# felipeagc/sycl-ray-tracer

Hardware: AMD Instinct MI355X
Metric: Mrays/s (higher is better)
Workload: dtype f32

## Files before the change

### include/rt_mi355x.h

```cpp
#ifndef RT_MI355X_H
#define RT_MI355X_H

#include <stddef.h>
#include <stdint.h>

#ifdef __cplusplus
extern "C" {
#endif

#define RT_ABI_VERSION 8

typedef enum rt_status {
    RT_OK = 0,
    RT_ERR_INVALID = -1,
    RT_ERR_NO_DEVICE = -2,
    RT_ERR_HIP = -3,
    RT_ERR_OOM = -4,
    RT_ERR_UNSUPPORTED = -5
} rt_status;

#define RT_TEX_SIZE 512u
#define RT_TEX_CHANNELS 4u
#define RT_TEX_MAX_LAYERS 128u

// ... 432 lines not shown
const void* rt_comm_frame_f32(const rt_comm* c);
const void* rt_comm_frame_u8(const rt_comm* c);

int rt_probe_xorshift(int device, uint32_t seed, uint32_t n, float* out, uint32_t* state_out);
int rt_probe_half_roundtrip(int device, uint32_t n, const float* in, float* out,
                            uint16_t* bits_out);
int rt_probe_scatter(rt_scene* scene, uint32_t material, uint32_t n, const float* dir,
                     const float* normal, const float* uv, const uint32_t* seed, uint8_t* ok,
                     float* out_dir, float* out_att, uint32_t* seed_out);

int rt_probe_rounding(int device, uint64_t* mismatches);

int rt_probe_origin_skip(int device, uint32_t n, const uint32_t* entries, const float* org, const float* dir,
                         uint32_t* word_device, uint32_t* word_host);

const char* rt_last_error(void);
int rt_abi_version(void);
int rt_device_count(void);

#ifdef __cplusplus
}
#endif
#endif
```

### sycl-ray-tracer_amd/csrc/rt_bounce.h

```cpp
#pragma once
#include "rt_device.h"

namespace rt {

RT_DEV f3 ray_dir(const RayState& r) { return mk3(h2f(r.dir[0]), h2f(r.dir[1]), h2f(r.dir[2])); }

template <bool FROM_TRAV = false, class Sink = NoSink>
RT_DEV bool shade_bounce(const SceneDev& S, uint32_t& rng, RayState& r, const Hit& h, f3& result, const Trav* T = nullptr, const ShadeTables* tab = nullptr,
                         long long* ck = nullptr, const Sink& sink = Sink{}) {
    f3 org = FROM_TRAV ? T->o : r.org;
    f3 dir = FROM_TRAV ? T->d : ray_dir(r);
    f3 att = mk3(h2f(r.att[0]), h2f(r.att[1]), h2f(r.att[2]));
    f3 rad = mk3(h2f(r.rad[0]), h2f(r.rad[1]), h2f(r.rad[2]));
    const bool done = FROM_TRAV ? shade_hit<true>(S, *tab, rng, h, org, dir, att, rad, result, ck, sink) : shade_hit<false>(S, ShadeTables{}, rng, h, org, dir, att, rad, result, nullptr, sink);
    r.org = org;
    r.dir[0] = f2h(dir.x), r.dir[1] = f2h(dir.y), r.dir[2] = f2h(dir.z);
    r.att[0] = f2h(att.x), r.att[1] = f2h(att.y), r.att[2] = f2h(att.z);
    r.rad[0] = f2h(rad.x), r.rad[1] = f2h(rad.y), r.rad[2] = f2h(rad.z);
    return done;
}

RT_DEV void origin_skip_none(const TravStack& stack) { *lds_at(skip_word_addr(stack)) = (int32_t)kSkipNone; }
RT_DEV SkipRec skip_entry(const SkipRec* at) {
    const u32x4* ep = reinterpret_cast<const u32x4*>(at);
    const u32x4 a = ep[0], b = ep[1];
    SkipRec e;
    e.ref = a.x, e.n[0] = __uint_as_float(a.y), e.n[1] = __uint_as_float(a.z), e.n[2] = __uint_as_float(a.w);
    e.p[0] = __uint_as_float(b.x), e.p[1] = __uint_as_float(b.y), e.p[2] = __uint_as_float(b.z), e.a = b.w;
    return e;
}
RT_DEV void origin_skip(const SceneDev& S, uint32_t tri, const Trav& T, const TravStack& stack) {
    const SkipRec e = skip_entry(S.skip + (tri == kNoTri ? 0u : tri));
    const float o[3] = {T.o.x, T.o.y, T.o.z}, d[3] = {T.d.x, T.d.y, T.d.z};
    const uint32_t w = origin_skip_word(e, o, d);
    *lds_at(skip_word_addr(stack)) = (int32_t)(tri == kNoTri ? kSkipNone : w);
}

RT_DEV bool roulette(uint32_t& rng, RayState& r) {
    const float qx = h2f(r.att[0]), qy = h2f(r.att[1]), qz = h2f(r.att[2]);
    const float p = __builtin_fminf(__builtin_fmaxf(__builtin_fmaxf(qx, __builtin_fmaxf(qy, qz)), 0.05f), 1.0f);
    const float u = rng_next(rng);
    if (!(u < p)) return false;
    r.att[0] = f2h(qx / p), r.att[1] = f2h(qy / p), r.att[2] = f2h(qz / p);
    return true;
}

}
```

### sycl-ray-tracer_amd/csrc/rt_device.h

```cpp
#pragma once
#include <hip/hip_runtime.h>

#include "../../include/rt_mi355x.h"
#include "rt_types.h"

namespace rt {

#define RT_DEV __device__ __forceinline__

struct f3 {
    float x, y, z;
};
RT_DEV f3 mk3(float x, float y, float z) { return f3{x, y, z}; }
RT_DEV f3 operator+(f3 a, f3 b) { return mk3(a.x + b.x, a.y + b.y, a.z + b.z); }
RT_DEV f3 operator-(f3 a, f3 b) { return mk3(a.x - b.x, a.y - b.y, a.z - b.z); }
RT_DEV f3 operator-(f3 a) { return mk3(-a.x, -a.y, -a.z); }
RT_DEV f3 operator*(f3 a, f3 b) { return mk3(a.x * b.x, a.y * b.y, a.z * b.z); }
RT_DEV f3 operator*(float s, f3 a) { return mk3(s * a.x, s * a.y, s * a.z); }
RT_DEV f3 operator*(f3 a, float s) { return mk3(a.x * s, a.y * s, a.z * s); }
RT_DEV float dot3(f3 a, f3 b) { return (a.x * b.x + a.y * b.y) + a.z * b.z; }
RT_DEV f3 cross3(f3 a, f3 b) {
    return mk3(a.y * b.z - a.z * b.y, a.z * b.x - a.x * b.z, a.x * b.y - a.y * b.x);
}
RT_DEV float rcp_rn(float x) {
// ... 132 lines not shown

constexpr int32_t kTravDone = (int32_t)0x80000000;
#if defined(RT_DEVELOPER_KNOBS) && defined(RT_VOTE_INNER) && defined(RT_VOTE_LEAF)
constexpr uint32_t kVoteInner = RT_VOTE_INNER, kVoteLeaf = RT_VOTE_LEAF;
#else
constexpr uint32_t kVoteInner = 3u, kVoteLeaf = 4u;
#endif
struct Trav {
    f3 o, d;
    float ix, iy, iz;
    float ox, oy, oz;
    Hit best;
    int32_t cur;
    uint32_t sp;
};

struct TravStack;
RT_DEV uint32_t stack_base(const TravStack& st);
RT_DEV void trav_begin(Trav& T, f3 o, f3 d, const TravStack& st) {
    T.o = o, T.d = d;
    T.best.t = __builtin_huge_valf();
    T.best.u = T.best.v = 0.0f;
    T.best.tri = kNoTri;
    const float kTiny = 1e-30f;
    const float dx = __builtin_fabsf(d.x) < kTiny ? __builtin_copysignf(kTiny, d.x) : d.x;
    const float dy = __builtin_fabsf(d.y) < kTiny ? __builtin_copysignf(kTiny, d.y) : d.y;
    const float dz = __builtin_fabsf(d.z) < kTiny ? __builtin_copysignf(kTiny, d.z) : d.z;
    T.ix = __builtin_amdgcn_rcpf(dx), T.iy = __builtin_amdgcn_rcpf(dy), T.iz = __builtin_amdgcn_rcpf(dz);
    T.ox = -o.x * T.ix, T.oy = -o.y * T.iy, T.oz = -o.z * T.iz;
    T.cur = 0;
// ... 66 lines not shown

struct TravSigns {
    lmask nx, ny, nz;
};

RT_DEV float ub0(uint32_t w) { return (float)(w & 0xffu); }
RT_DEV float ub1(uint32_t w) { return (float)((w >> 8) & 0xffu); }
RT_DEV float ub2(uint32_t w) { return (float)((w >> 16) & 0xffu); }
RT_DEV float ub3(uint32_t w) { return (float)(w >> 24); }

struct WaveStats {
    uint32_t inner_steps = 0, inner_lanes = 0, leaf_steps = 0, leaf_lanes = 0;
    uint32_t shade_rounds = 0, shade_lanes = 0, live_lane_steps = 0, top_lanes = 0;
};
RT_DEV TravSigns trav_signs(const Trav& T) { return TravSigns{lanes(T.ix < 0.0f), lanes(T.iy < 0.0f), lanes(T.iz < 0.0f)}; }
template <bool SKIP = false, bool MISS_KEYS = false>
RT_DEV void trav_inner(const SceneDev& S, Trav& T, const TravStack& stack, const TopTree& top, const TravSigns& sg) {
    const float inf = __builtin_huge_valf();
    uint32_t skip = kSkipNone;
    if (SKIP) skip = (uint32_t)*lds_at(skip_word_addr(stack));
    float k0, k1, k2, k3;
    u32x4 w0, w1, w2, chw;
    if (T.cur < top.count * 64) {
        const uint32_t o = (uint32_t)T.cur >> 2;
        w0 = *(lds_u32x4*)(size_t)((uint32_t)(size_t)top.w0 + o), w1 = *(lds_u32x4*)(size_t)((uint32_t)(size_t)top.w1 + o);
        w2 = *(lds_u32x4*)(size_t)((uint32_t)(size_t)top.w2 + o), chw = *(lds_u32x4*)(size_t)((uint32_t)(size_t)top.ch + o);
    } else {
        asm volatile("global_load_dwordx4 %0, %4, %5\n\t"
                     "global_load_dwordx4 %1, %4, %5 offset:16\n\t"
                     "global_load_dwordx4 %2, %4, %5 offset:32\n\t"
                     "global_load_dwordx4 %3, %4, %5 offset:48"
                     : "=&v"(w0), "=&v"(w1), "=&v"(w2), "=&v"(chw)
                     : "v"((uint32_t)T.cur), "s"(S.nodes)
                     : "memory");
    }
// ... 111 lines not shown
        tri_test(S.tris + (size_t)first * kTriBytes, T.o, T.d, T.best);
        if (rem) T.cur = ~(int32_t)(((first + 1u) << 2) | (rem - 1u));
        else trav_pop(T, stack);
    }
}

struct TravClasses {
    lmask inner, leaf;
};
RT_DEV lmask trav_done(const Trav& T) { return lanes(T.cur == kTravDone); }
RT_DEV TravClasses trav_classes(const Trav& T) { return TravClasses{lanes(T.cur >= 0), lanes((uint32_t)T.cur > (uint32_t)kTravDone)}; }
RT_DEV TravClasses trav_classes(const Trav& T, lmask done) {
    const lmask inner = lanes(T.cur >= 0);
    return TravClasses{inner, lanes(true) & ~(inner | done)};
}
template <bool STATS = false, bool LEAF_BATCH = false, bool SKIP = false, bool MISS_KEYS = false>
RT_DEV uint32_t trav_step_wave(const SceneDev& S, Trav& T, const TravStack& stack, const TopTree& top, const TravSigns& sg, const TravClasses& c, WaveStats* ws = nullptr) {
    const uint32_t ni = count(c.inner), nl = count(c.leaf);
    if (ni * kVoteInner >= nl * kVoteLeaf && !(LEAF_BATCH && nl >= 64u)) {
        if (STATS && ni) ws->inner_steps++, ws->inner_lanes += ni, ws->top_lanes += count(c.inner & lanes(T.cur < (SKIP ? top.count : kTopNodes) * 64));
        if (in_mask(c.inner)) trav_inner<SKIP, MISS_KEYS>(S, T, stack, top, sg);
    } else {
        if (STATS) ws->leaf_steps++, ws->leaf_lanes += nl;
        if (in_mask(c.leaf)) trav_leaf<LEAF_BATCH>(S, T, stack);
    }
    return ni + nl;
}
template <bool STATS = false, bool LEAF_BATCH = false, bool SKIP = false, bool MISS_KEYS = false>
RT_DEV uint32_t trav_step_wave(const SceneDev& S, Trav& T, const TravStack& stack, const TopTree& top, const TravSigns& sg, WaveStats* ws = nullptr) {
    return trav_step_wave<STATS, LEAF_BATCH, SKIP, MISS_KEYS>(S, T, stack, top, sg, trav_classes(T), ws);
}

RT_DEV Hit intersect(const SceneDev& S, f3 o, f3 d, const TravStack& stack, const TopTree& top) {
    Trav T;
    trav_begin(T, o, d, stack);
    const TravSigns sg = trav_signs(T);
    while (trav_step_wave(S, T, stack, top, sg)) {}
    return T.best;
}

RT_DEV bool near_zero3(f3 e) {
    const float s = 1e-8f;
    return (__builtin_fabsf(e.x) < s) && (__builtin_fabsf(e.y) < s) && (__builtin_fabsf(e.z) < s);
}
RT_DEV float length_squared3(f3 v) {
// ... 240 lines not shown
```

### sycl-ray-tracer_amd/csrc/rt_frame.hip

```cpp
#include "rt_internal.h"
#include "rt_kernels.h"



namespace rtlib {

void drop_graph(rt_renderer* r) {
    if (r->graph_exec) (void)hipGraphExecDestroy(r->graph_exec);
    r->graph_exec = nullptr;
}

void free_block_state(rt_renderer* r) {
    if (r->d_blk) (void)hipFree(r->d_blk);
    if (r->d_snap) (void)hipFree(r->d_snap);
    if (r->h_blk) (void)hipHostFree(r->h_blk);
    r->d_blk = nullptr, r->d_snap = nullptr, r->h_blk = nullptr;
    r->blocks_x = r->blocks_y = 0;
    r->h_block_count.clear();
}
size_t blk_words(const rt_renderer* r) { return std::max<size_t>((size_t)r->blocks_x * r->blocks_y, 1); }
int alloc_block_state(rt_renderer* r) {
    free_block_state(r);
    if (!r->d_carry) return RT_OK;
    r->blocks_x = ((uint32_t)r->width + 7u) / 8u, r->blocks_y = ((uint32_t)r->tile.local_rows + 7u) / 8u;
// ... 643 lines not shown
    if (r->n_local == 0) {
        if (stats) stats->launches = 0, stats->pixel_slices = 1;
        return RT_OK;
    }
    const bool blocks = p.req.carry == kCarryBlocks;
    if (r->kind == RT_RENDERER_MEGAKERNEL) {
        HIPCHK(hipMemsetAsync(r->d_ray_counter, 0, 8 * sizeof(unsigned long long), st));
        hipEvent_t e0 = pool_event(r->ev_pool, 0), e1 = pool_event(r->ev_pool, 1);
        if (!e0 || !e1) return fail(RT_ERR_HIP, "hipEventCreate failed");
        SliceDev sl = p.sl;
        if (int rc_ = next_slice_tag(r, p.req.spp, st, &sl)) return rc_;
        r->h_frame->cam = c, r->h_frame->sl = sl;
        r->h_frame->carry = r->d_carry, r->h_frame->carry_total = p.req.carry_total;
        r->h_frame->n_blocks = blocks ? p.req.n_blocks : 0u;
        r->h_frame->seed_add = frame_seed_add(r);
        r->h_frame->blocks = r->d_blk ? r->d_blk + 5 * blk_words(r) + 1 : nullptr, r->h_frame->block_count = r->d_blk;
        HIPCHK(hipMemcpyAsync(r->d_frame, r->h_frame, sizeof(MegaFrame), hipMemcpyHostToDevice, st));
        if (blocks && r->max_depth > 0 && (d_f32 || d_u8)) {
            hipLaunchKernelGGL(k_blocks_resolve, dim3((r->n_local + 255u) / 256u), dim3(256), 0, st, r->n_local, (uint32_t)r->width, r->blocks_x,
                               (const u32x4*)r->d_carry, (const uint32_t*)r->d_blk, d_f32, d_u8);
            launches.add(RT_K_BLOCK_RESOLVE);
        }
        HIPCHK(hipEventRecord(e0, st));
        if (r->max_depth == 0) {
            hipLaunchKernelGGL(k_fill_black, dim3((r->n_local + 255u) / 256u), dim3(256), 0, st, r->n_local, d_f32, d_u8);
            launches.add(p.hot);
        } else if (!blocks || p.req.n_blocks) {
            if (r->d_stats) {
                HIPCHK(hipMemsetAsync(r->d_stats, 0, 13 * sizeof(unsigned long long), st));
                HIPCHK(hipMemsetAsync(r->d_stats + 13, 0xff, 2 * sizeof(unsigned long long), st));
// ... 386 lines not shown
```

### sycl-ray-tracer_amd/csrc/rt_kernels.h

```cpp
#pragma once
#include <cstddef>

#include "rt_bounce.h"
#include "rt_device.h"
#include "rt_launch.h"

namespace rt {

RT_DEV void queue_store(const QueueDev& q, uint32_t slot, uint32_t id, const RayState& r) {
    q.org_id[slot] = make_float4(r.org.x, r.org.y, r.org.z, __uint_as_float(id));
    q.a[slot] = make_uint2((uint32_t)r.dir[0] | ((uint32_t)r.dir[1] << 16), (uint32_t)r.dir[2] | ((uint32_t)r.att[0] << 16));
    q.b[slot] = make_uint2((uint32_t)r.att[1] | ((uint32_t)r.att[2] << 16), (uint32_t)r.rad[0] | ((uint32_t)r.rad[1] << 16));
    q.c[slot] = r.rad[2];
}
RT_DEV uint32_t queue_load(const QueueDev& q, uint32_t slot, RayState& r) {
    const float4 o = q.org_id[slot];
    const uint2 a = q.a[slot], b = q.b[slot];
    const uint16_t c = q.c[slot];
    r.org = mk3(o.x, o.y, o.z);
    r.dir[0] = (uint16_t)a.x, r.dir[1] = (uint16_t)(a.x >> 16), r.dir[2] = (uint16_t)a.y;
    r.att[0] = (uint16_t)(a.y >> 16), r.att[1] = (uint16_t)b.x, r.att[2] = (uint16_t)(b.x >> 16);
    r.rad[0] = (uint16_t)b.y, r.rad[1] = (uint16_t)(b.y >> 16), r.rad[2] = c;
    return __float_as_uint(o.w);
}
// ... 100 lines not shown
                 "s_load_dwordx4 %1, %4, 0x10\n\t"
                 "s_load_dwordx4 %2, %4, 0x20\n\t"
                 "s_load_dword %3, %4, %5\n\t"
                 "s_waitcnt lgkmcnt(0)"
                 : "=&s"(a), "=&s"(b), "=&s"(c), "=&s"(s)
                 : "s"(f), "i"((uint32_t)offsetof(MegaFrame, seed_add)));
    CameraDev cam;
    cam.center[0] = __uint_as_float(a.x), cam.center[1] = __uint_as_float(a.y), cam.center[2] = __uint_as_float(a.z);
    cam.pixel00[0] = __uint_as_float(a.w), cam.pixel00[1] = __uint_as_float(b.x), cam.pixel00[2] = __uint_as_float(b.y);
    cam.du[0] = __uint_as_float(b.z), cam.du[1] = __uint_as_float(b.w), cam.du[2] = __uint_as_float(c.x);
    cam.dv[0] = __uint_as_float(c.y), cam.dv[1] = __uint_as_float(c.z), cam.dv[2] = __uint_as_float(c.w);
    cam.width = width, cam.height = height;
    seed_add = s;
    return cam;
}
struct SliceNow {
    u32x4 head;
    u32x2 cuts;
};
RT_DEV SliceNow frame_slices(const MegaFrame* f) {
    static_assert(offsetof(SliceDev, tag0) == offsetof(SliceDev, state) + 8 && offsetof(SliceDev, shift) == offsetof(SliceDev, state) + 12, "SliceNow::head");
    SliceNow n;
    asm volatile("s_load_dwordx4 %0, %2, %3\n\t"
                 "s_load_dwordx2 %1, %2, %4\n\t"
                 "s_waitcnt lgkmcnt(0)"
                 : "=&s"(n.head), "=&s"(n.cuts)
                 : "s"(f), "i"((uint32_t)offsetof(MegaFrame, sl.state)), "i"((uint32_t)offsetof(MegaFrame, sl.cuts)));
    return n;
}
RT_DEV uint32_t frame_slice_bound(const MegaFrame* f, uint32_t j) {
// ... 34 lines not shown
__global__ void __launch_bounds__(kMegaBlock, kMegaWaves) k_megakernel(SceneDev S, const MegaFrame* frame, int32_t width, int32_t height, TileDev tile,
                                                    uint32_t max_depth, uint32_t spp, uint32_t seed_mode, uint32_t rr_start, float* __restrict__ out_f32,
                                                    uint8_t* __restrict__ out_u8,
                                                    unsigned long long* __restrict__ ray_counter,
                                                    unsigned long long* __restrict__ stats_out, uint32_t n_slices) {
    WaveStats ws;
    long long t_begin = 0, t_mark = 0, t_trav = 0, t_shade = 0;
    long long ck[8] = {0, 0, 0, 0, 0, 0, 0, 0};
    if (STATS) t_begin = t_mark = (long long)__builtin_readcyclecounter();
    unsigned long long wall_begin = 0, wall_exhausted = 0;
    if (STATS >= 2) wall_begin = wall_clock64();
    const uint32_t tiles_x = (uint32_t)(width + 7) >> 3, tiles_y = (uint32_t)(tile.local_rows + 7) >> 3;
    const uint32_t n_slots = (CARRY == 3 ? frame_n_blocks(frame) : tiles_x * tiles_y) * 64u;
    const int lane = (int)(threadIdx.x & 63u);
    uint32_t* pixel_cursor = reinterpret_cast<uint32_t*>(ray_counter + 1);
    int x = 0, gy = 0;
    uint32_t pix = 0;
    uint32_t rng = 0, s = 0, depth = 0;
    unsigned long long wave_rays = 0;
    __shared__ float color_lds[3 * kMegaBlock + (SLICED ? kMegaBlock / 64 : 0)];
    typedef __attribute__((address_space(3))) float lds_f32;
    lds_f32* const color_r = (lds_f32*)color_lds + threadIdx.x;
    lds_f32* const color_g = color_r + kMegaBlock;
    lds_f32* const color_b = color_g + kMegaBlock;
    RayState r{};
    Trav T;
    if (SLICED) *slice_looks_word(color_r, (lds_f32*)color_lds) = 0u;
    RT_SHADE_LDS
    RT_TRAVERSAL_LDS_SKIP(kMegaBlock, true)
    T.cur = kTravDone;
    constexpr uint32_t kPend = 0x40000000u;
    bool live = false;
    RefillPolicy<kMegaUnroll> refill;
    bool exhausted = false;
    uint32_t slice_j = 0;
    auto state_rsrc = [&](const SliceNow& n) {
        return __builtin_amdgcn_make_buffer_rsrc((void*)(((unsigned long long)n.head.y << 32) | n.head.x), 0, (int)((uint32_t)tile.local_rows * (uint32_t)width * 32u), 0x00020000);
    };
    auto take_slot = [&](uint32_t p, uint32_t first) {
        uint32_t t = p >> 6;
        if constexpr (CARRY == 3) t = frame_blocks(frame)[t];
        x = (int)((t % tiles_x) * 8u + (p & 7u));
        const int ly = (int)((t / tiles_x) * 8u + ((p >> 3) & 7u));
        gy = tile_global_row(tile, ly);
        pix = (uint32_t)ly * (uint32_t)width + (uint32_t)x;
        if (x < width && ly < tile.local_rows && gy < height) {
            s = first;
            if (!SLICED || first == 0) {
                depth = 0;
                if constexpr (CARRY >= 2) {
                    const u32x4 c = frame_carry(frame)[pix];
                    rng = c.w;
                    *color_r = __uint_as_float(c.x), *color_g = __uint_as_float(c.y), *color_b = __uint_as_float(c.z);
                    r = camera_ray(frame_camera(frame, width, height), x, gy, rng);
                } else {
                    uint32_t seed_add;
                    const CameraDev cam = frame_camera_and_seed(frame, width, height, seed_add);
                    rng = pixel_seed(x, gy, width, height, seed_mode) + seed_add;
                    *color_r = 0.0f, *color_g = 0.0f, *color_b = 0.0f;
                    r = camera_ray(cam, x, gy, rng);
                }
                trav_begin(T, r.org, ray_dir(r), stack);
                origin_skip_none(stack);
            } else {
                depth = kPend;
            }
            live = true;
        }
    };
    {
        const uint32_t n_waves = gridDim.x * (kMegaBlock / 64u);
        if (n_slots <= n_waves * 64u && n_slices == 1u) {
            const uint32_t p = (uint32_t)lane * n_waves + blockIdx.x * (kMegaBlock / 64u) + (threadIdx.x >> 6);
            if (p < n_slots) take_slot(p, 0u);
            exhausted = true;
            if (STATS >= 2) wall_exhausted = wall_clock64();
        }
    }
    for (;;) {
        if (!exhausted) {
// ... 18 lines not shown
                    take_slot(m.slot, m.first);
                }
                if (base + w >= total_slots) {
                    exhausted = true;
                    if (STATS >= 2) wall_exhausted = wall_clock64();
                }
            }
        }
        const uint32_t n_live = (uint32_t)__popcll(__ballot(live));
        if (n_live == 0) {
            if (exhausted) break;
            continue;
        }
        if (STATS) t_mark = (long long)__builtin_readcyclecounter();
        const TravSigns sg = trav_signs(T);
        const uint32_t n_rays = SLICED ? (uint32_t)__popcll(__ballot(live && depth < kPend)) : n_live;
        const lmask live_m = lanes(live);
        const uint32_t shade_at = n_rays * kMegaShadePct + (n_live - n_rays) * 100u;
        for (;;) {
            const lmask done = trav_done(T);
            if (count(done & live_m) * 100u >= shade_at) break;
            if (STATS >= 2) ws.live_lane_steps += n_live * (uint32_t)kMegaUnroll;
            if (STATS == 1) ws.inner_steps += (uint32_t)kMegaUnroll;
            refill.stepped();
            (void)trav_step_wave<(STATS >= 2), true, true, true>(S, T, stack, top, sg, trav_classes(T, done), &ws);
#pragma unroll
            for (int k = 1; k < kMegaUnroll; ++k) (void)trav_step_wave<(STATS >= 2), true, true, true>(S, T, stack, top, sg, &ws);
        }
        if (STATS) {
            ws.shade_rounds++;
            if (STATS >= 2) ws.shade_lanes += (uint32_t)__popcll(__ballot(live && T.cur == kTravDone));
            const long long now = (long long)__builtin_readcyclecounter();
            t_trav += now - t_mark, t_mark = now;
        }
        __builtin_amdgcn_s_setprio(RT_ROUND_PRIO);
#ifdef RT_ROUND_STAMPS
        if (STATS >= 2) ck[7] = (long long)__builtin_readcyclecounter();
#endif
        bool pixel_finished = false;
        bool bounced = false;
        {
            const unsigned long long traced = __ballot(live && T.cur == kTravDone && depth < kPend);
            wave_rays += (unsigned long long)__popcll(traced);
            if (SLICED && traced == 0ull && __ballot(live && depth < kPend) == 0ull && slice_wait_count(slice_looks_word(color_r, (lds_f32*)color_lds), frame) && lane == 0) atomicMax(ray_counter + 2, 1ull);
        }
        if (live && T.cur == kTravDone) {
            bool start = false;
            if (SLICED && depth >= kPend) {
                const SliceNow sn = frame_slices(frame);
                const auto rsrc = state_rsrc(sn);
                const uint32_t at = pix * 32u, tag = sn.head.z + s;
                const u32x4 w0 = __builtin_amdgcn_raw_buffer_load_b128(rsrc, (int)at, 0, 16 );
                const u32x4 w1 = __builtin_amdgcn_raw_buffer_load_b128(rsrc, (int)(at + 16u), 0, 16 );
                if ((w0.y == tag && w0.w == tag && w1.y == tag && w1.w == tag) || slice_wait_over(slice_looks_word(color_r, (lds_f32*)color_lds), frame)) {
                    *color_r = __uint_as_float(w0.x), *color_g = __uint_as_float(w0.z), *color_b = __uint_as_float(w1.x);
                    rng = w1.z;
                    start = true;
                }
            } else {
                f3 res;
                const auto add = [color_r, color_g, color_b](const f3& c) { *color_r = *color_r + c.x, *color_g = *color_g + c.y, *color_b = *color_b + c.z; };
                bool done;
                if (SLICED) {
                    done = shade_bounce<true>(S, rng, r, T.best, res, &T, &tab, STATS >= 2 ? ck : nullptr, add);
                } else {
                    done = shade_bounce<true>(S, rng, r, T.best, res, &T, &tab, STATS >= 2 ? ck : nullptr);
                    if (done) add(res);
                }
#ifdef RT_TAIL_PRIO
                __builtin_amdgcn_s_setprio(RT_TAIL_PRIO);
#endif
                depth++;
                bool killed = false;
                if (rr_start && !done && depth >= rr_start && depth < max_depth) killed = !roulette(rng, r);
                if (done || killed || depth == max_depth) {
                    s++;
                    bool handed = false;
                    SliceNow sn{};
                    if (SLICED) {
                        sn = frame_slices(frame);
                        const unsigned long long cuts = ((unsigned long long)sn.cuts.y << 32) | sn.cuts.x;
                        const uint32_t sh = sn.head.w;
                        handed = s < spp && (s & ((1u << sh) - 1u)) == 0u && ((cuts >> (s >> sh)) & 1ull) != 0ull;
                    }
                    if (SLICED && handed) {
                        live = false, pixel_finished = true;
                        const auto rsrc = state_rsrc(sn);
                        const uint32_t at = pix * 32u, tag = sn.head.z + s;
                        u32x4 w0, w1;
                        w0.x = __float_as_uint(*color_r), w0.y = tag, w0.z = __float_as_uint(*color_g), w0.w = tag;
                        w1.x = __float_as_uint(*color_b), w1.y = tag, w1.z = rng, w1.w = tag;
                        __builtin_amdgcn_raw_buffer_store_b128(w0, rsrc, (int)at, 0, 16 );
                        __builtin_amdgcn_raw_buffer_store_b128(w1, rsrc, (int)(at + 16u), 0, 16 );
                    } else if (s < spp) {
                        start = true;
                    } else {
                        live = false, pixel_finished = true;
                        float n;
                        if constexpr (CARRY == 3)
                            n = (float)frame_block_count(frame)[(pix / (uint32_t)width >> 3) * tiles_x + ((uint32_t)x >> 3)];
                        else
                            n = (float)(CARRY == 2 ? frame_carry_total(frame) : spp);
                        pixel_end(color_r, color_g, color_b, n, pix, out_f32, out_u8);
                        if constexpr (CARRY != 0) frame_carry(frame)[pix] = carry_word(*color_r, *color_g, *color_b, rng);
                    }
                } else {
                    bounced = true;
                }
            }
            if (start) {
                depth = 0;
                int cx = x, cy = gy;
                asm volatile("" : "+v"(cx), "+v"(cy));
                r = camera_ray(frame_camera(frame, width, height), cx, cy, rng);
            }
            if (live && depth < kPend) {
                const uint32_t from = bounced ? T.best.tri : kNoTri;
                trav_begin(T, r.org, ray_dir(r), stack);
                origin_skip(S, from, T, stack);
            }
            RT_STAMP_AFTER((STATS >= 2 ? ck : nullptr), 5, T.ox);
        }
        refill.round(pixel_finished);
        if (STATS) t_shade += (long long)__builtin_readcyclecounter() - t_mark;
        __builtin_amdgcn_s_setprio(2);
    }
    if (lane == 0 && wave_rays) atomicAdd(ray_counter, wave_rays);
    if (STATS && lane == 0) {
        wave_stats_flush(ws, stats_out);
        const unsigned long long dur = (unsigned long long)((long long)__builtin_readcyclecounter() - t_begin);
        atomicAdd(stats_out + 8, dur), atomicMax(stats_out + 9, dur), atomicAdd(stats_out + 10, 1ull);
        atomicAdd(stats_out + 11, (unsigned long long)t_trav), atomicAdd(stats_out + 12, (unsigned long long)t_shade);
        if (STATS >= 2) {
            atomicMin(stats_out + 13, wall_begin);
// ... 836 lines not shown
```

### sycl-ray-tracer_amd/csrc/rt_launch.h

```cpp
#pragma once
#include <hip/hip_runtime.h>

#include <cstddef>
#include <cstdint>

#include "rt_types.h"

namespace rt {


struct QueueDev {
    float4* org_id;
    uint2* a;
    uint2* b;
    uint16_t* c;
};


constexpr uint32_t kMegaBlock = 512;
constexpr uint32_t kMegaWaves = 6;

constexpr uint32_t kMaxSlices = 8;
struct SliceDev {
    void* state;
// ... 9 lines not shown
    uint32_t slot;
    uint32_t first;
};
struct SliceCursor {
    __host__ __device__ __forceinline__ static uint32_t claim_width(uint32_t idle, uint32_t n) { return idle < n ? idle : n; }
    __host__ __device__ __forceinline__ static uint32_t advance(uint32_t slice_j, uint32_t n_slices, uint32_t pos, uint32_t n) {
        while (slice_j + 1u < n_slices && pos >= (slice_j + 1u) * n) slice_j++;
        return slice_j;
    }
    __host__ __device__ __forceinline__ static SliceSlot map(uint32_t q, uint32_t slice_j, uint32_t n, uint32_t first_here, uint32_t first_next) {
        const uint32_t p = q - slice_j * n;
        const bool next = p >= n;
        return SliceSlot{next ? p - n : p, next ? first_next : first_here};
    }
};
struct MegaFrame {
    CameraDev cam;
    SliceDev sl;
    void* carry;
    uint32_t carry_total;
    uint32_t n_blocks;
    const uint32_t* blocks;
    const uint32_t* block_count;
    uint32_t seed_add;
};

constexpr uint32_t kExtendChunk = 128;
constexpr uint32_t kExtendBlock = 1024;
constexpr uint32_t kExtendWaves = 8;

struct FinishRequeue {
    unsigned long long* entries;
    uint32_t* ctl;
    uint32_t* error;
    uint32_t capacity;
};

constexpr uint32_t kOutBlock = 256u;

// ... 2 lines not shown
```

### sycl-ray-tracer_amd/csrc/rt_probes.hip

```cpp
#include "rt_internal.h"
#include "rt_probe_kernels.h"

extern "C" {

int rt_intersect_batch(rt_scene* s, uint32_t n, const float* org, const float* dir, float* t, float* u, float* v,
                       uint32_t* tri) {
    if (!s || (n && (!org || !dir || !t || !u || !v || !tri))) return fail(RT_ERR_INVALID, "null argument");
    if (s->device < 0) return fail(RT_ERR_NO_DEVICE, "scene was built host-only (device < 0)");
    if (n == 0) return RT_OK;
    for (uint32_t i = 0; i < n; ++i)
        if (!origin_in_contract_range(s->hs, org + 3 * (size_t)i))
            return fail(RT_ERR_INVALID, "ray " + std::to_string(i) + ": origin more than 100 scene scales outside the scene's bounds (outside the range of the closest-hit contract)");
    HIPCHK(hipSetDevice(s->device));
    DevBuf b_org, b_dir, b_out;
    HIPCHK(b_org.alloc((size_t)n * 12));
    HIPCHK(b_dir.alloc((size_t)n * 12));
    HIPCHK(b_out.alloc((size_t)n * 16));
    float *d_org = b_org.as<float>(), *d_dir = b_dir.as<float>(), *d_out = b_out.as<float>();
    HIPCHK(hipMemcpy(d_org, org, (size_t)n * 12, hipMemcpyHostToDevice));
    HIPCHK(hipMemcpy(d_dir, dir, (size_t)n * 12, hipMemcpyHostToDevice));
    float* d_t = d_out;
    float* d_u = d_out + n;
    float* d_v = d_out + 2 * (size_t)n;
    uint32_t* d_tri = (uint32_t*)(d_out + 3 * (size_t)n);
    hipLaunchKernelGGL(k_intersect_batch, dim3((n + 255u) / 256u), dim3(256), 0, 0, s->dev, n, d_org, d_dir, d_t, d_u, d_v, d_tri);
    HIPCHK(hipGetLastError());
    HIPCHK(hipDeviceSynchronize());
    HIPCHK(hipMemcpy(t, d_t, (size_t)n * 4, hipMemcpyDeviceToHost));
    HIPCHK(hipMemcpy(u, d_u, (size_t)n * 4, hipMemcpyDeviceToHost));
    HIPCHK(hipMemcpy(v, d_v, (size_t)n * 4, hipMemcpyDeviceToHost));
    HIPCHK(hipMemcpy(tri, d_tri, (size_t)n * 4, hipMemcpyDeviceToHost));
    return RT_OK;
}

}

extern "C" {

int rt_probe_xorshift(int device, uint32_t seed, uint32_t n, float* out, uint32_t* state_out) {
    if (!out || !state_out || n == 0) return fail(RT_ERR_INVALID, "bad arguments");
    int rc = device_ok(device);
    if (rc != RT_OK) return rc;
    DevBuf b_out, b_st;
    HIPCHK(b_out.alloc((size_t)n * 4));
    HIPCHK(b_st.alloc(4));
    hipLaunchKernelGGL(k_probe_xorshift, dim3(1), dim3(64), 0, 0, seed, n, b_out.as<float>(), b_st.as<uint32_t>());
// ... 104 lines not shown
```

### sycl-ray-tracer_amd/rtamd/abi.py

```python
from __future__ import annotations

import ctypes as C
import os
from pathlib import Path

PKG_DIR = Path(__file__).resolve().parent.parent
REPO_DIR = PKG_DIR.parent
LIB_PATH = PKG_DIR / "csrc" / "build" / "librt_mi355x.so"

RT_OK = 0
RT_ERR_INVALID, RT_ERR_NO_DEVICE, RT_ERR_HIP, RT_ERR_OOM, RT_ERR_UNSUPPORTED = -1, -2, -3, -4, -5

RT_MAT_NONE, RT_MAT_DIFFUSE, RT_MAT_METALLIC, RT_MAT_DIELECTRIC = 0, 1, 2, 3
RT_TEX_COLOR, RT_TEX_IMAGE = 0, 1
RT_RENDERER_MEGAKERNEL, RT_RENDERER_WAVEFRONT = 0, 1
RT_SEED_DEFAULT, RT_SEED_WAVEFRONT, RT_SEED_MEGAKERNEL = 0, 1, 2
RT_BVH_DEFAULT, RT_BVH_LBVH, RT_BVH_SAH, RT_BVH_LBVH_GPU = 0, 1, 2, 3
RT_BVH_MEDIAN_INTERNAL = 99
RT_SCENE_UPDATABLE = 1
RT_SCENE_KEEP_PREVIOUS = 2
RT_TEX_SIZE = 512
RT_TEX_MAX_LAYERS = 128


# ... 507 lines not shown
    "rt_renderer_tile_u8": (C.c_void_p, [C.c_void_p]),
    "rt_frame_gather": (C.c_int, [C.c_void_p, _P(C.c_void_p), _P(C.c_float), _P(C.c_uint8), C.c_int, C.c_int]),
    "rt_frame_gather_begin": (C.c_int, [C.c_void_p, _P(C.c_void_p), C.c_int, C.c_int]),
    "rt_comm_wait": (C.c_int, [C.c_void_p, _P(C.c_float), _P(C.c_uint8)]),
    "rt_comm_size": (C.c_int, [C.c_void_p]),
    "rt_comm_frame_f32": (C.c_void_p, [C.c_void_p]),
    "rt_comm_frame_u8": (C.c_void_p, [C.c_void_p]),
    "rt_probe_xorshift": (C.c_int, [C.c_int, C.c_uint32, C.c_uint32, _P(C.c_float), _P(C.c_uint32)]),
    "rt_probe_half_roundtrip": (C.c_int, [C.c_int, C.c_uint32, _P(C.c_float), _P(C.c_float), _P(C.c_uint16)]),
    "rt_probe_scatter": (C.c_int, [C.c_void_p, C.c_uint32, C.c_uint32, _P(C.c_float), _P(C.c_float),
                                   _P(C.c_float), _P(C.c_uint32), _P(C.c_uint8), _P(C.c_float),
                                   _P(C.c_float), _P(C.c_uint32)]),
    "rt_last_error": (C.c_char_p, []),
    "rt_probe_rounding": (C.c_int, [C.c_int, _P(C.c_uint64)]),
    "rt_probe_origin_skip": (C.c_int, [C.c_int, C.c_uint32, _P(C.c_uint32), _P(C.c_float), _P(C.c_float), _P(C.c_uint32), _P(C.c_uint32)]),
    "rt_abi_version": (C.c_int, []),
    "rt_device_count": (C.c_int, []),
}

_lib = None


class RtError(RuntimeError):
    def __init__(self, status: int, msg: str):
        super().__init__(f"rt_status {status}: {msg}")
        self.status = status


def load_library(path: os.PathLike | None = None) -> C.CDLL:
    global _lib
# ... 69 lines not shown
```

Baseline: 10750.

## Cut megakernel per-lane register state: pack sample/depth, recompute pixel coords, keep skip word in registers

The megakernel no longer keeps x and gy live across the loop. When a new sample starts it recomputes them from the pixel index, using host-precomputed magic-number division constants that are loaded together with the camera in one scalar load batch. The sample counter and bounce depth are packed into one word, and the origin-skip word moves from LDS into a register field of the traversal state. The aim is lower VGPR pressure and less LDS traffic, possibly raising occupancy. The cost is extra integer math on restart and new validation limits on frame size and spp.

```diff
diff --git a/include/rt_mi355x.h b/include/rt_mi355x.h
--- a/include/rt_mi355x.h
+++ b/include/rt_mi355x.h
@@ -470,6 +470,10 @@
 int rt_probe_origin_skip(int device, uint32_t n, const uint32_t* entries, const float* org, const float* dir,
                          uint32_t* word_device, uint32_t* word_host);
 
+int rt_probe_pixel_index(uint32_t width, uint32_t rank, uint32_t world, uint32_t strip_rows, uint64_t pix_begin, uint64_t pix_end, uint32_t n,
+                         const uint32_t* pix, uint64_t* mismatches, uint32_t* constants);
+int rt_probe_sample_word(uint64_t spp, uint64_t max_depth, uint32_t* bits, uint32_t* fits);
+
 const char* rt_last_error(void);
 int rt_abi_version(void);
 int rt_device_count(void);
diff --git a/sycl-ray-tracer_amd/csrc/rt_bounce.h b/sycl-ray-tracer_amd/csrc/rt_bounce.h
--- a/sycl-ray-tracer_amd/csrc/rt_bounce.h
+++ b/sycl-ray-tracer_amd/csrc/rt_bounce.h
@@ -35,6 +35,13 @@
     const uint32_t w = origin_skip_word(e, o, d);
     *lds_at(skip_word_addr(stack)) = (int32_t)(tri == kNoTri ? kSkipNone : w);
 }
+RT_DEV void origin_skip_none(TravSkip& T) { T.skip = kSkipNone; }
+RT_DEV void origin_skip(const SceneDev& S, uint32_t tri, TravSkip& T) {
+    const SkipRec e = skip_entry(S.skip + (tri == kNoTri ? 0u : tri));
+    const float o[3] = {T.o.x, T.o.y, T.o.z}, d[3] = {T.d.x, T.d.y, T.d.z};
+    const uint32_t w = origin_skip_word(e, o, d);
+    T.skip = tri == kNoTri ? kSkipNone : w;
+}
 
 RT_DEV bool roulette(uint32_t& rng, RayState& r) {
     const float qx = h2f(r.att[0]), qy = h2f(r.att[1]), qz = h2f(r.att[2]);
diff --git a/sycl-ray-tracer_amd/csrc/rt_device.h b/sycl-ray-tracer_amd/csrc/rt_device.h
--- a/sycl-ray-tracer_amd/csrc/rt_device.h
+++ b/sycl-ray-tracer_amd/csrc/rt_device.h
@@ -170,6 +170,9 @@
     int32_t cur;
     uint32_t sp;
 };
+struct TravSkip : Trav {
+    uint32_t skip;
+};
 
 struct TravStack;
 RT_DEV uint32_t stack_base(const TravStack& st);
@@ -266,11 +269,12 @@
     uint32_t shade_rounds = 0, shade_lanes = 0, live_lane_steps = 0, top_lanes = 0;
 };
 RT_DEV TravSigns trav_signs(const Trav& T) { return TravSigns{lanes(T.ix < 0.0f), lanes(T.iy < 0.0f), lanes(T.iz < 0.0f)}; }
-template <bool SKIP = false, bool MISS_KEYS = false>
-RT_DEV void trav_inner(const SceneDev& S, Trav& T, const TravStack& stack, const TopTree& top, const TravSigns& sg) {
+template <bool SKIP = false, bool MISS_KEYS = false, bool SKIP_REG = false, class TRAV = Trav>
+RT_DEV void trav_inner(const SceneDev& S, TRAV& T, const TravStack& stack, const TopTree& top, const TravSigns& sg) {
     const float inf = __builtin_huge_valf();
     uint32_t skip = kSkipNone;
-    if (SKIP) skip = (uint32_t)*lds_at(skip_word_addr(stack));
+    if constexpr (SKIP_REG) skip = T.skip;
+    else if (SKIP) skip = (uint32_t)*lds_at(skip_word_addr(stack));
     float k0, k1, k2, k3;
     u32x4 w0, w1, w2, chw;
     if (T.cur < top.count * 64) {
@@ -412,21 +416,21 @@
     const lmask inner = lanes(T.cur >= 0);
     return TravClasses{inner, lanes(true) & ~(inner | done)};
 }
-template <bool STATS = false, bool LEAF_BATCH = false, bool SKIP = false, bool MISS_KEYS = false>
-RT_DEV uint32_t trav_step_wave(const SceneDev& S, Trav& T, const TravStack& stack, const TopTree& top, const TravSigns& sg, const TravClasses& c, WaveStats* ws = nullptr) {
+template <bool STATS = false, bool LEAF_BATCH = false, bool SKIP = false, bool MISS_KEYS = false, bool SKIP_REG = false, class TRAV = Trav>
+RT_DEV uint32_t trav_step_wave(const SceneDev& S, TRAV& T, const TravStack& stack, const TopTree& top, const TravSigns& sg, const TravClasses& c, WaveStats* ws = nullptr) {
     const uint32_t ni = count(c.inner), nl = count(c.leaf);
     if (ni * kVoteInner >= nl * kVoteLeaf && !(LEAF_BATCH && nl >= 64u)) {
         if (STATS && ni) ws->inner_steps++, ws->inner_lanes += ni, ws->top_lanes += count(c.inner & lanes(T.cur < (SKIP ? top.count : kTopNodes) * 64));
-        if (in_mask(c.inner)) trav_inner<SKIP, MISS_KEYS>(S, T, stack, top, sg);
+        if (in_mask(c.inner)) trav_inner<SKIP, MISS_KEYS, SKIP_REG>(S, T, stack, top, sg);
     } else {
         if (STATS) ws->leaf_steps++, ws->leaf_lanes += nl;
         if (in_mask(c.leaf)) trav_leaf<LEAF_BATCH>(S, T, stack);
     }
     return ni + nl;
 }
-template <bool STATS = false, bool LEAF_BATCH = false, bool SKIP = false, bool MISS_KEYS = false>
-RT_DEV uint32_t trav_step_wave(const SceneDev& S, Trav& T, const TravStack& stack, const TopTree& top, const TravSigns& sg, WaveStats* ws = nullptr) {
-    return trav_step_wave<STATS, LEAF_BATCH, SKIP, MISS_KEYS>(S, T, stack, top, sg, trav_classes(T), ws);
+template <bool STATS = false, bool LEAF_BATCH = false, bool SKIP = false, bool MISS_KEYS = false, bool SKIP_REG = false, class TRAV = Trav>
+RT_DEV uint32_t trav_step_wave(const SceneDev& S, TRAV& T, const TravStack& stack, const TopTree& top, const TravSigns& sg, WaveStats* ws = nullptr) {
+    return trav_step_wave<STATS, LEAF_BATCH, SKIP, MISS_KEYS, SKIP_REG>(S, T, stack, top, sg, trav_classes(T), ws);
 }
 
 RT_DEV Hit intersect(const SceneDev& S, f3 o, f3 d, const TravStack& stack, const TopTree& top) {
diff --git a/sycl-ray-tracer_amd/csrc/rt_frame.hip b/sycl-ray-tracer_amd/csrc/rt_frame.hip
--- a/sycl-ray-tracer_amd/csrc/rt_frame.hip
+++ b/sycl-ray-tracer_amd/csrc/rt_frame.hip
@@ -681,6 +681,11 @@
         r->h_frame->carry = r->d_carry, r->h_frame->carry_total = p.req.carry_total;
         r->h_frame->n_blocks = blocks ? p.req.n_blocks : 0u;
         r->h_frame->seed_add = frame_seed_add(r);
+        const uint32_t strip_div = std::min(r->tile.strip_rows, kPixDivLimit);
+        if (!pix_div_ok((uint64_t)c.width, r->n_local) || !pix_div_ok(strip_div, (uint64_t)std::max(r->tile.local_rows, 0)) ||
+            (r->max_depth > 0 && !sample_depth_ok(p.req.spp, r->max_depth)))
+            return fail(RT_ERR_INVALID, "frame outside the megakernel's pixel-index or sample-word range");
+        r->h_frame->px = PixIndex{pix_div_make((uint32_t)c.width), pix_div_make(strip_div)};
         r->h_frame->blocks = r->d_blk ? r->d_blk + 5 * blk_words(r) + 1 : nullptr, r->h_frame->block_count = r->d_blk;
         HIPCHK(hipMemcpyAsync(r->d_frame, r->h_frame, sizeof(MegaFrame), hipMemcpyHostToDevice, st));
         if (blocks && r->max_depth > 0 && (d_f32 || d_u8)) {
diff --git a/sycl-ray-tracer_amd/csrc/rt_kernels.h b/sycl-ray-tracer_amd/csrc/rt_kernels.h
--- a/sycl-ray-tracer_amd/csrc/rt_kernels.h
+++ b/sycl-ray-tracer_amd/csrc/rt_kernels.h
@@ -138,6 +138,29 @@
     seed_add = s;
     return cam;
 }
+RT_DEV CameraDev frame_camera_and_place(const MegaFrame* f, int32_t width, int32_t height, PixIndex& px) {
+    static_assert(offsetof(MegaFrame, px) % 16 == 0 && sizeof(PixIndex) == 16, "PixIndex is one 16-byte load");
+    u32x4 a, b, c, d;
+    asm volatile("s_load_dwordx4 %0, %4, 0x0\n\t"
+                 "s_load_dwordx4 %1, %4, 0x10\n\t"
+                 "s_load_dwordx4 %2, %4, 0x20\n\t"
+                 "s_load_dwordx4 %3, %4, %5\n\t"
+                 "s_waitcnt lgkmcnt(0)"
+                 : "=&s"(a), "=&s"(b), "=&s"(c), "=&s"(d)
+                 : "s"(f), "i"((uint32_t)offsetof(MegaFrame, px)));
+    CameraDev cam;
+    cam.center[0] = __uint_as_float(a.x), cam.center[1] = __uint_as_float(a.y), cam.center[2] = __uint_as_float(a.z);
+    cam.pixel00[0] = __uint_as_float(a.w), cam.pixel00[1] = __uint_as_float(b.x), cam.pixel00[2] = __uint_as_float(b.y);
+    cam.du[0] = __uint_as_float(b.z), cam.du[1] = __uint_as_float(b.w), cam.du[2] = __uint_as_float(c.x);
+    cam.dv[0] = __uint_as_float(c.y), cam.dv[1] = __uint_as_float(c.z), cam.dv[2] = __uint_as_float(c.w);
+    cam.width = width, cam.height = height;
+    px.width = PixDiv{d.x, d.y}, px.strip = PixDiv{d.z, d.w};
+    return cam;
+}
+RT_DEV PixDiv frame_width_div(const MegaFrame* f) {
+    const unsigned long long v = frame_u64<offsetof(MegaFrame, px.width)>(f);
+    return PixDiv{(uint32_t)v, (uint32_t)(v >> 32)};
+}
 struct SliceNow {
     u32x4 head;
     u32x2 cuts;
@@ -202,9 +225,10 @@
     const uint32_t n_slots = (CARRY == 3 ? frame_n_blocks(frame) : tiles_x * tiles_y) * 64u;
     const int lane = (int)(threadIdx.x & 63u);
     uint32_t* pixel_cursor = reinterpret_cast<uint32_t*>(ray_counter + 1);
-    int x = 0, gy = 0;
     uint32_t pix = 0;
-    uint32_t rng = 0, s = 0, depth = 0;
+    const uint32_t dbits = depth_bits(max_depth);
+    const auto depth_of = [dbits](uint32_t w) { return w & ((1u << dbits) - 1u); };
+    uint32_t rng = 0, sd = 0;
     unsigned long long wave_rays = 0;
     __shared__ float color_lds[3 * kMegaBlock + (SLICED ? kMegaBlock / 64 : 0)];
     typedef __attribute__((address_space(3))) float lds_f32;
@@ -212,11 +236,12 @@
     lds_f32* const color_g = color_r + kMegaBlock;
     lds_f32* const color_b = color_g + kMegaBlock;
     RayState r{};
-    Trav T;
+    TravSkip T;
     if (SLICED) *slice_looks_word(color_r, (lds_f32*)color_lds) = 0u;
     RT_SHADE_LDS
-    RT_TRAVERSAL_LDS_SKIP(kMegaBlock, true)
+    RT_TRAVERSAL_LDS(kMegaBlock)
     T.cur = kTravDone;
+    T.skip = kSkipNone;
     constexpr uint32_t kPend = 0x40000000u;
     bool live = false;
     RefillPolicy<kMegaUnroll> refill;
@@ -228,14 +253,13 @@
     auto take_slot = [&](uint32_t p, uint32_t first) {
         uint32_t t = p >> 6;
         if constexpr (CARRY == 3) t = frame_blocks(frame)[t];
-        x = (int)((t % tiles_x) * 8u + (p & 7u));
+        const int x = (int)((t % tiles_x) * 8u + (p & 7u));
         const int ly = (int)((t / tiles_x) * 8u + ((p >> 3) & 7u));
-        gy = tile_global_row(tile, ly);
+        const int gy = tile_global_row(tile, ly);
         pix = (uint32_t)ly * (uint32_t)width + (uint32_t)x;
         if (x < width && ly < tile.local_rows && gy < height) {
-            s = first;
+            sd = first << dbits;
             if (!SLICED || first == 0) {
-                depth = 0;
                 if constexpr (CARRY >= 2) {
                     const u32x4 c = frame_carry(frame)[pix];
                     rng = c.w;
@@ -249,9 +273,9 @@
                     r = camera_ray(cam, x, gy, rng);
                 }
                 trav_begin(T, r.org, ray_dir(r), stack);
-                origin_skip_none(stack);
+                origin_skip_none(T);
             } else {
-                depth = kPend;
+                sd |= kPend;
             }
             live = true;
         }
@@ -300,7 +324,7 @@
         }
         if (STATS) t_mark = (long long)__builtin_readcyclecounter();
         const TravSigns sg = trav_signs(T);
-        const uint32_t n_rays = SLICED ? (uint32_t)__popcll(__ballot(live && depth < kPend)) : n_live;
+        const uint32_t n_rays = SLICED ? (uint32_t)__popcll(__ballot(live && sd < kPend)) : n_live;
         const lmask live_m = lanes(live);
         const uint32_t shade_at = n_rays * kMegaShadePct + (n_live - n_rays) * 100u;
         for (;;) {
@@ -309,9 +333,9 @@
             if (STATS >= 2) ws.live_lane_steps += n_live * (uint32_t)kMegaUnroll;
             if (STATS == 1) ws.inner_steps += (uint32_t)kMegaUnroll;
             refill.stepped();
-            (void)trav_step_wave<(STATS >= 2), true, true, true>(S, T, stack, top, sg, trav_classes(T, done), &ws);
+            (void)trav_step_wave<(STATS >= 2), true, true, false, true>(S, T, stack, top, sg, trav_classes(T, done), &ws);
 #pragma unroll
-            for (int k = 1; k < kMegaUnroll; ++k) (void)trav_step_wave<(STATS >= 2), true, true, true>(S, T, stack, top, sg, &ws);
+            for (int k = 1; k < kMegaUnroll; ++k) (void)trav_step_wave<(STATS >= 2), true, true, false, true>(S, T, stack, top, sg, &ws);
         }
         if (STATS) {
             ws.shade_rounds++;
@@ -326,21 +350,22 @@
         bool pixel_finished = false;
         bool bounced = false;
         {
-            const unsigned long long traced = __ballot(live && T.cur == kTravDone && depth < kPend);
+            const unsigned long long traced = __ballot(live && T.cur == kTravDone && sd < kPend);
             wave_rays += (unsigned long long)__popcll(traced);
-            if (SLICED && traced == 0ull && __ballot(live && depth < kPend) == 0ull && slice_wait_count(slice_looks_word(color_r, (lds_f32*)color_lds), frame) && lane == 0) atomicMax(ray_counter + 2, 1ull);
+            if (SLICED && traced == 0ull && __ballot(live && sd < kPend) == 0ull && slice_wait_count(slice_looks_word(color_r, (lds_f32*)color_lds), frame) && lane == 0) atomicMax(ray_counter + 2, 1ull);
         }
         if (live && T.cur == kTravDone) {
             bool start = false;
-            if (SLICED && depth >= kPend) {
+            if (SLICED && sd >= kPend) {
                 const SliceNow sn = frame_slices(frame);
                 const auto rsrc = state_rsrc(sn);
-                const uint32_t at = pix * 32u, tag = sn.head.z + s;
+                const uint32_t at = pix * 32u, tag = sn.head.z + ((sd - kPend) >> dbits);
                 const u32x4 w0 = __builtin_amdgcn_raw_buffer_load_b128(rsrc, (int)at, 0, 16 );
                 const u32x4 w1 = __builtin_amdgcn_raw_buffer_load_b128(rsrc, (int)(at + 16u), 0, 16 );
                 if ((w0.y == tag && w0.w == tag && w1.y == tag && w1.w == tag) || slice_wait_over(slice_looks_word(color_r, (lds_f32*)color_lds), frame)) {
                     *color_r = __uint_as_float(w0.x), *color_g = __uint_as_float(w0.z), *color_b = __uint_as_float(w1.x);
                     rng = w1.z;
+                    sd -= kPend;
                     start = true;
                 }
             } else {
@@ -356,11 +381,13 @@
 #ifdef RT_TAIL_PRIO
                 __builtin_amdgcn_s_setprio(RT_TAIL_PRIO);
 #endif
-                depth++;
+                sd++;
+                const uint32_t depth = depth_of(sd);
                 bool killed = false;
                 if (rr_start && !done && depth >= rr_start && depth < max_depth) killed = !roulette(rng, r);
                 if (done || killed || depth == max_depth) {
-                    s++;
+                    const uint32_t s = (sd >> dbits) + 1u;
+                    sd = s << dbits;
                     bool handed = false;
                     SliceNow sn{};
                     if (SLICED) {
@@ -384,7 +411,11 @@
                         live = false, pixel_finished = true;
                         float n;
                         if constexpr (CARRY == 3)
-                            n = (float)frame_block_count(frame)[(pix / (uint32_t)width >> 3) * tiles_x + ((uint32_t)x >> 3)];
+                        {
+                            const PixDiv wd = frame_width_div(frame);
+                            const uint32_t ly = pix_div(pix, wd.magic, wd.shift);
+                            n = (float)frame_block_count(frame)[(ly >> 3) * tiles_x + ((pix - ly * (uint32_t)width) >> 3)];
+                        }
                         else
                             n = (float)(CARRY == 2 ? frame_carry_total(frame) : spp);
                         pixel_end(color_r, color_g, color_b, n, pix, out_f32, out_u8);
@@ -395,15 +426,15 @@
                 }
             }
             if (start) {
-                depth = 0;
-                int cx = x, cy = gy;
-                asm volatile("" : "+v"(cx), "+v"(cy));
-                r = camera_ray(frame_camera(frame, width, height), cx, cy, rng);
-            }
-            if (live && depth < kPend) {
+                PixIndex px;
+                const CameraDev cam = frame_camera_and_place(frame, width, height, px);
+                const PixPlace at = pix_place(pix, (uint32_t)width, tile, px);
+                r = camera_ray(cam, (int)at.x, (int)at.gy, rng);
+            }
+            if (live && sd < kPend) {
                 const uint32_t from = bounced ? T.best.tri : kNoTri;
                 trav_begin(T, r.org, ray_dir(r), stack);
-                origin_skip(S, from, T, stack);
+                origin_skip(S, from, T);
             }
             RT_STAMP_AFTER((STATS >= 2 ? ck : nullptr), 5, T.ox);
         }
diff --git a/sycl-ray-tracer_amd/csrc/rt_launch.h b/sycl-ray-tracer_amd/csrc/rt_launch.h
--- a/sycl-ray-tracer_amd/csrc/rt_launch.h
+++ b/sycl-ray-tracer_amd/csrc/rt_launch.h
@@ -47,6 +47,40 @@
         return SliceSlot{next ? p - n : p, next ? first_next : first_here};
     }
 };
+
+struct PixDiv {
+    uint32_t magic, shift;
+};
+constexpr uint32_t kPixDivLimit = 1u << 31;
+inline bool pix_div_ok(uint64_t divisor, uint64_t dividend_end) { return divisor >= 1 && divisor <= kPixDivLimit && dividend_end <= kPixDivLimit; }
+inline PixDiv pix_div_make(uint32_t d) {
+    uint32_t L = 0;
+    while (L < 31u && (1u << L) < d) L++;
+    return PixDiv{(uint32_t)(((1ull << (31u + L)) + d - 1u) / d), L};
+}
+__host__ __device__ __forceinline__ uint32_t pix_div(uint32_t n, uint32_t magic, uint32_t shift) {
+    return (uint32_t)(((unsigned long long)(n << 1) * magic) >> 32) >> shift;
+}
+struct alignas(16) PixIndex {
+    PixDiv width, strip;
+};
+struct PixPlace {
+    uint32_t x, ly, gy;
+};
+__host__ __device__ __forceinline__ PixPlace pix_place(uint32_t pix, uint32_t width, const TileDev& t, const PixIndex& px) {
+    PixPlace p;
+    p.ly = pix_div(pix, px.width.magic, px.width.shift);
+    p.x = pix - p.ly * width;
+    const uint32_t strip = pix_div(p.ly, px.strip.magic, px.strip.shift);
+    p.gy = (strip * t.world + t.rank) * t.strip_rows + (p.ly - strip * t.strip_rows);
+    return p;
+}
+constexpr uint32_t kSampleDepthBits = 27;
+__host__ __device__ __forceinline__ uint32_t depth_bits(uint32_t max_depth) { return 32u - (uint32_t)__builtin_clz(max_depth | 1u); }
+inline bool sample_depth_ok(uint64_t spp, uint64_t max_depth) {
+    return max_depth < (1ull << 31) && (spp << depth_bits((uint32_t)max_depth)) < (1ull << kSampleDepthBits) && max_depth < (1ull << depth_bits((uint32_t)max_depth));
+}
+
 struct MegaFrame {
     CameraDev cam;
     SliceDev sl;
@@ -56,6 +90,7 @@
     const uint32_t* blocks;
     const uint32_t* block_count;
     uint32_t seed_add;
+    PixIndex px;
 };
 
 constexpr uint32_t kExtendChunk = 128;
diff --git a/sycl-ray-tracer_amd/csrc/rt_probes.hip b/sycl-ray-tracer_amd/csrc/rt_probes.hip
--- a/sycl-ray-tracer_amd/csrc/rt_probes.hip
+++ b/sycl-ray-tracer_amd/csrc/rt_probes.hip
@@ -30,6 +30,40 @@
     HIPCHK(hipMemcpy(u, d_u, (size_t)n * 4, hipMemcpyDeviceToHost));
     HIPCHK(hipMemcpy(v, d_v, (size_t)n * 4, hipMemcpyDeviceToHost));
     HIPCHK(hipMemcpy(tri, d_tri, (size_t)n * 4, hipMemcpyDeviceToHost));
+    return RT_OK;
+}
+
+int rt_probe_pixel_index(uint32_t width, uint32_t rank, uint32_t world, uint32_t strip_rows, uint64_t pix_begin, uint64_t pix_end, uint32_t n,
+                         const uint32_t* pix, uint64_t* mismatches, uint32_t* constants) {
+    if (!mismatches || (n && !pix) || world == 0 || rank >= world || strip_rows == 0 || pix_begin > pix_end) return fail(RT_ERR_INVALID, "bad arguments");
+    if (!pix_div_ok(width, pix_end)) return fail(RT_ERR_INVALID, "width or pixel index outside the range the reciprocal is proved for (2^31)");
+    const TileDev tile{rank, world, strip_rows, 0};
+    const PixIndex px{pix_div_make(width), pix_div_make(std::min(strip_rows, kPixDivLimit))};
+    if (constants) constants[0] = px.width.magic, constants[1] = px.width.shift, constants[2] = px.strip.magic, constants[3] = px.strip.shift;
+    uint64_t bad = 0;
+    uint32_t ly = (uint32_t)(pix_begin / width), x = (uint32_t)(pix_begin % width), strip = ly / strip_rows, within = ly % strip_rows;
+    for (uint64_t i = pix_begin; i < pix_end; ++i) {
+        const PixPlace p = pix_place((uint32_t)i, width, tile, px);
+        bad += p.ly != ly || p.x != x || p.gy != (strip * world + rank) * strip_rows + within;
+        if (++x == width) {
+            x = 0, ++ly;
+            if (++within == strip_rows) within = 0, ++strip;
+        }
+    }
+    for (uint32_t i = 0; i < n; ++i) {
+        if (pix[i] >= kPixDivLimit) return fail(RT_ERR_INVALID, "pixel index outside the range the reciprocal is proved for (2^31)");
+        const PixPlace p = pix_place(pix[i], width, tile, px);
+        const uint32_t row = pix[i] / width;
+        bad += p.ly != row || p.x != pix[i] % width || p.gy != (row / strip_rows * world + rank) * strip_rows + row % strip_rows;
+    }
+    *mismatches = bad;
+    return RT_OK;
+}
+
+int rt_probe_sample_word(uint64_t spp, uint64_t max_depth, uint32_t* bits, uint32_t* fits) {
+    if (!bits || !fits || max_depth >= (1ull << 31)) return fail(RT_ERR_INVALID, "bad arguments");
+    *bits = depth_bits((uint32_t)max_depth);
+    *fits = sample_depth_ok(spp, max_depth) ? 1u : 0u;
     return RT_OK;
 }
 
diff --git a/sycl-ray-tracer_amd/rtamd/abi.py b/sycl-ray-tracer_amd/rtamd/abi.py
--- a/sycl-ray-tracer_amd/rtamd/abi.py
+++ b/sycl-ray-tracer_amd/rtamd/abi.py
@@ -545,6 +545,8 @@
     "rt_last_error": (C.c_char_p, []),
     "rt_probe_rounding": (C.c_int, [C.c_int, _P(C.c_uint64)]),
     "rt_probe_origin_skip": (C.c_int, [C.c_int, C.c_uint32, _P(C.c_uint32), _P(C.c_float), _P(C.c_float), _P(C.c_uint32), _P(C.c_uint32)]),
+    "rt_probe_pixel_index": (C.c_int, [C.c_uint32, C.c_uint32, C.c_uint32, C.c_uint32, C.c_uint64, C.c_uint64, C.c_uint32, _P(C.c_uint32), _P(C.c_uint64), _P(C.c_uint32)]),
+    "rt_probe_sample_word": (C.c_int, [C.c_uint64, C.c_uint64, _P(C.c_uint32), _P(C.c_uint32)]),
     "rt_abi_version": (C.c_int, []),
     "rt_device_count": (C.c_int, []),
 }
```

After: 10800, median of 6. Within noise of the previous version (+0.5%).
